# Juleszwanen/oscar_mpc_planner_mr_modification

Hardware: AMD Instinct MI355X
Metric: SQP solves/s (N=20, 8 obs, 8 guesses) at 1/2/4/8 MI355X; max |x−x_ref| (higher is better)
Workload: dtype f64

## Files before the change

__graft_entry__.py:

```python
import os
import sys

ROOT = os.path.dirname(os.path.abspath(__file__))
if ROOT not in sys.path:
    sys.path.insert(0, ROOT)


def build() -> None:
    from oscar_mpc_planner_mr_modification_amd import _build

    _build.build_lib()
    for cfg in ("C2", "C5", "C3", "JS"):
        _build.build_cpp(cfg)
    from oscar_mpc_planner_mr_modification_amd.layouts import tmpc_layout
    _build.build_instance(tmpc_layout(N=25, max_obstacles=3, name="G25"), os.path.join(_build.BUILD, "G25"))
    _build.build_stage_probe()
    _build.build_mirror_probe()
    _build.build_fac_rows_probe()
    for name in _build.FAC_AB:
        _build.build_fac_ab(name)
    _build.build_tail_ab("tail_off")
    sys.path.insert(0, os.path.join(ROOT, "oracle"))
    import oracle_py

    oracle_py.build()
    import oscar_mpc_planner_mr_modification_amd
    from oscar_mpc_planner_mr_modification_amd import native


def smoke() -> None:
    import numpy as np
    import torch

    sys.path.insert(0, os.path.join(ROOT, "oracle"))
    import oracle_py
    from oscar_mpc_planner_mr_modification_amd import native
    from oscar_mpc_planner_mr_modification_amd.layouts import config_layout
    from oscar_mpc_planner_mr_modification_amd.synthetic import make_batch

    assert torch.cuda.is_available(), "smoke() needs an MI355X"
    dev = torch.device("cuda:0")
    lay = config_layout("C2")
    b = make_batch(lay, 2, 8, seed=20251212)
    pr = native.problem_from_layout(lay)
    t = lambda a: torch.from_numpy(np.ascontiguousarray(a)).to(dev)
    out = native.solve_batch_device(pr, t(b.params), t(b.warm), t(b.xinit))
    torch.cuda.synchronize()
    ref = oracle_py.Oracle(lay).solve_batch(b.params, b.warm, b.xinit)
    exit_gpu = out["exit"].cpu().numpy()
    assert np.array_equal(exit_gpu, ref["status"]), (exit_gpu, ref["status"])
    ok = exit_gpu == 1
    assert ok.any()
    dx = np.abs(out["xtraj"].cpu().numpy()[ok] - ref["xtraj"][ok]).max()
    assert dx <= 1e-4, dx
    print(f"smoke ok: {len(exit_gpu)} solves, {int(ok.sum())} successful, max|x-x_ref| = {dx:.2e}")


if __name__ == "__main__":
    build()
    if len(sys.argv) > 1 and sys.argv[1] == "smoke":
        smoke()
```

oscar_mpc_planner_mr_modification_amd/_build.py:

```python
from __future__ import annotations

import os
import subprocess

PKG = os.path.dirname(os.path.abspath(__file__))
ROOT = os.path.dirname(PKG)
CSRC = os.path.join(PKG, "csrc")
INCLUDE = os.path.join(ROOT, "include")
LIB = os.path.join(PKG, "libmpcg.so")
ARCH = os.environ.get("MPCG_OFFLOAD_ARCH", "gfx950")

SOURCES = {"mpcg_kernels.hip": [], "mpcg_prepare.hip": ["-ffp-contract=off"],
           "mpcg_inst_tmpc20.hip": [], "mpcg_inst_tmpc30.hip": [], "mpcg_inst_shmpc.hip": [],
           "mpcg_inst_bicycle.hip": [], "mpcg_inst_road.hip": []}
HEADERS = ["mpcg_device.h", "mpcg_sqp.h", "mpcg_sqp_body.inc", "mpcg_prepare.h", "mpcg_braking.h", "mpcg_bicycle.h",
           "mpcg_instance.h", "mpcg_tail.h"]
LAYERS = {
    "mpcg_fleet.h": {"sources": {"mpcg_fleet.hip": ["-ffp-contract=off"]}, "headers": ["mpcg_fleet.h"]},
    "mpcg_path.h": {"sources": {"mpcg_path.hip": ["-ffp-contract=off"]}, "headers": ["mpcg_path.h"]},
    "mpcg_guidance.h": {"sources": {"mpcg_guidance.hip": ["-ffp-contract=off"]}, "headers": ["mpcg_guidance.h"]},
    "mpcg_active.h": {"sources": {"mpcg_active.hip": ["-ffp-contract=off"]}, "headers": ["mpcg_active.h"]},
    "mpcg_road.h": {"sources": {"mpcg_road.hip": ["-ffp-contract=off"]}, "headers": ["mpcg_road.h"]},
}
LAYER_SHARED_HEADERS = ["mpcg_host.h", "mpcg_spline.h"]
HOST_SOURCES = ["host/mpcg_yaml.cpp", "host/mpcg_solver.cpp"]
HOST_HEADERS = ["mpc_planner_solver/mpcg_yaml.h", "mpc_planner_solver/mpcg_config.h", "mpc_planner_solver/state.h",
                "mpc_planner_solver/mpcg_solver_interface.h", "mpc_planner_solver/solver_interface.h"]
BUILD = os.path.join(PKG, "build")


def source_hash() -> str:
    import hashlib

    h = hashlib.sha256()
    for f in sorted(list(SOURCES) + HEADERS):
        h.update(f.encode())
        with open(os.path.join(CSRC, f), "rb") as fh:
            h.update(fh.read())
    with open(os.path.join(INCLUDE, "mpcg.h"), "rb") as fh:
        h.update(fh.read())
    h.update(repr((ARCH, sorted(SOURCES.items()))).encode())
    return h.hexdigest()


def _stale(target, deps):
    if not os.path.exists(target):
        return True
    t = os.path.getmtime(target)
    return any(os.path.getmtime(d) > t for d in deps)


def lib_sources() -> dict:
    srcs = dict(SOURCES)
    for layer in LAYERS.values():
        srcs.update(layer["sources"])
    return srcs


def build_lib(force: bool = False, verbose: bool = False, extra_flags=(), out: str = LIB, sources=None) -> str:
    srcs = {k: v for k, v in lib_sources().items() if sources is None or k not in SOURCES or k in sources}
    layer_headers = LAYER_SHARED_HEADERS + [h for layer in LAYERS.values() for h in layer["headers"]]
    deps = [os.path.join(CSRC, f) for f in list(lib_sources()) + HEADERS + layer_headers] + \
        [os.path.join(INCLUDE, h) for h in ["mpcg.h"] + list(LAYERS)] + [__file__]
    if not force and not _stale(out, deps):
        return out
    objdir = os.path.join(BUILD, "obj" + ("_" + "_".join(f.strip("-").replace("=", "") for f in extra_flags)
                                          if extra_flags else ""))
    os.makedirs(objdir, exist_ok=True)
    common = ["hipcc", f"--offload-arch={ARCH}", "-O3", "-std=c++17", "-fPIC", f"-I{INCLUDE}", f"-I{CSRC}"]
    objs, procs = [], []
    for src, flags in srcs.items():
        obj = os.path.join(objdir, src.replace(".hip", ".o"))
        cmd = common + list(flags) + list(extra_flags) + ["-c", os.path.join(CSRC, src), "-o", obj]
        if verbose:
            print(" ".join(cmd))
        procs.append(subprocess.Popen(cmd))
        objs.append(obj)
    for p in procs:
        if p.wait() != 0:
            raise subprocess.CalledProcessError(p.returncode, "hipcc")
    cmd = ["hipcc", f"--offload-arch={ARCH}", "-shared", "-fPIC", "-Wl,-soname,libmpcg.so", "-o", out + ".tmp"] + objs
    if verbose:
        print(" ".join(cmd))
    subprocess.run(cmd, check=True)
    os.replace(out + ".tmp", out)
    return out


def _hipcc_obj(src, obj, extra=()):
    cmd = ["hipcc", f"--offload-arch={ARCH}", "-O3", "-std=c++17", "-fPIC", f"-I{INCLUDE}", f"-I{CSRC}",
           *extra, "-c", src, "-o", obj]
    subprocess.run(cmd, check=True)
    return obj


def build_instance(layout, out_dir: str, force: bool = False) -> str:
    from . import codegen

    lib_mpcg = build_lib()
    os.makedirs(out_dir, exist_ok=True)
    src = os.path.join(out_dir, "mpcg_instance.hip")
    text = codegen.instance_source(layout)
    if not os.path.exists(src) or open(src).read() != text:
        with open(src, "w") as fh:
            fh.write(text)
    so = os.path.join(out_dir, f"libmpcg_inst_{layout.name}.so")
    deps = [src, lib_mpcg, os.path.join(INCLUDE, "mpcg.h")] + [os.path.join(CSRC, h) for h in HEADERS]
    if force or _stale(so, deps):
        obj = _hipcc_obj(src, os.path.join(out_dir, "mpcg_instance.o"))
        subprocess.run(["hipcc", f"--offload-arch={ARCH}", "-shared", "-fPIC", "-o", so + ".tmp", obj, f"-L{PKG}",
                        "-lmpcg", f"-Wl,-rpath,{PKG}"], check=True)
        os.replace(so + ".tmp", so)
    return so


def _build_probe(name: str, headers, force: bool) -> str:
    src = os.path.join(ROOT, "tests", "cpp", name + ".hip")
    out_dir = os.path.join(BUILD, "probe")
    so = os.path.join(out_dir, f"lib{name}.so")
    deps = [src, os.path.join(INCLUDE, "mpcg.h"), __file__] + [os.path.join(CSRC, h) for h in headers]
    if force or _stale(so, deps):
        os.makedirs(out_dir, exist_ok=True)
        obj = _hipcc_obj(src, os.path.join(out_dir, name + ".o"))
        subprocess.run(["hipcc", f"--offload-arch={ARCH}", "-shared", "-fPIC", "-o", so + ".tmp", obj], check=True)
        os.replace(so + ".tmp", so)
    return so


def build_stage_probe(force: bool = False) -> str:
    return _build_probe("stage_probe", HEADERS, force)


def build_mirror_probe(force: bool = False) -> str:
    return _build_probe("mirror_probe", ["mpcg_device.h"], force)


def build_fac_rows_probe(force: bool = False) -> str:
    return _build_probe("fac_rows_probe", ["mpcg_device.h"], force)


FAC_AB = {"fac_rows0": ["-DMPCG_FAC_INVARIANT_ROWS=0"],
          "fac_off": ["-DMPCG_FAC_INVARIANT_ROWS=0", "-DMPCG_FAC_PIVOT_SELECT=0"]}


def build_fac_ab(name: str, force: bool = False) -> str:
    out = os.path.join(BUILD, "ab", name, "libmpcg.so")
    os.makedirs(os.path.dirname(out), exist_ok=True)
    return build_lib(force=force, extra_flags=FAC_AB[name], out=out,
                     sources=("mpcg_kernels.hip", "mpcg_prepare.hip", "mpcg_inst_tmpc20.hip"))


TAIL_AB = {"tail_off": ["-DMPCG_TAIL_LEVELS=0"], "tail_poison": ["-DMPCG_LEVEL_POISON"]}


def build_tail_ab(name: str = "tail_off", force: bool = False) -> str:
    out = os.path.join(BUILD, "ab", name, "libmpcg.so")
    os.makedirs(os.path.dirname(out), exist_ok=True)
    return build_lib(force=force, extra_flags=TAIL_AB[name], out=out,
                     sources=("mpcg_kernels.hip", "mpcg_prepare.hip", "mpcg_inst_tmpc20.hip"))


def build_cpp(config="C2", force: bool = False, verbose: bool = False) -> dict:
    from . import codegen
    from .layouts import config_layout

    lay = config_layout(config) if isinstance(config, str) else config
    lib_mpcg = build_lib()
    out = os.path.join(BUILD, lay.name)
    codegen.generate(lay, out)
    so = os.path.join(out, "libmpc_planner_solver.so")
    exe = os.path.join(out, "test_solver")
    srcs = [os.path.join(CSRC, s) for s in HOST_SOURCES] + [os.path.join(out, "mpc_planner_parameters.cpp")]
    inst = os.path.join(out, "mpcg_instance.hip")
    deps = srcs + [inst] + [os.path.join(INCLUDE, h) for h in HOST_HEADERS] + \
        [os.path.join(CSRC, h) for h in HEADERS] + [os.path.join(INCLUDE, "mpcg.h"), lib_mpcg, __file__]
    inc = [f"-I{os.path.join(out, 'include')}", f"-I{INCLUDE}"]
    if force or _stale(so, deps):
        objs = []
        for src in srcs:
            obj = os.path.join(out, os.path.basename(src).replace(".cpp", ".o"))
            cmd = ["g++", "-std=c++17", "-O2", "-fPIC", "-Wall", "-Wextra"] + inc + ["-c", src, "-o", obj]
            if verbose:
                print(" ".join(cmd))
            subprocess.run(cmd, check=True)
            objs.append(obj)
        objs.append(_hipcc_obj(inst, os.path.join(out, "mpcg_instance.o")))
        cmd = ["hipcc", f"--offload-arch={ARCH}", "-shared", "-fPIC"] + objs + \
              ["-o", so + ".tmp", f"-L{PKG}", "-lmpcg", f"-Wl,-rpath,{PKG}"]
        if verbose:
            print(" ".join(cmd))
        subprocess.run(cmd, check=True)
        os.replace(so + ".tmp", so)
    test_src = os.path.join(ROOT, "tests", "cpp", "test_solver.cpp")
    if os.path.exists(test_src) and (force or _stale(exe, [test_src, so])):
        cmd = ["g++", "-std=c++17", "-O2", "-Wall", "-Wextra"] + inc + [test_src, "-o", exe, f"-L{out}",
                                                                      "-lmpc_planner_solver", f"-L{PKG}", "-lmpcg",
                                                                      f"-Wl,-rpath,{out}:{PKG}"]
        if verbose:
            print(" ".join(cmd))
        subprocess.run(cmd, check=True)
    return {"dir": out, "lib": so, "test": exe}


if __name__ == "__main__":
    print(build_lib(force=True, verbose=True))
    print(build_cpp("C2", force=True, verbose=True))
```

oscar_mpc_planner_mr_modification_amd/csrc/mpcg_instance.h:

```cpp
#pragma once
#include <hip/hip_runtime.h>

#include <atomic>
#include <cstdio>

#include "mpcg.h"
#include "mpcg_sqp.h"

extern "C" {
typedef int (*mpcg_instance_launch)(const mpcg_problem* pr, int batch, const mpcg_io* io, void* stream,
                                    unsigned long long* stamps, void* workspace);
int mpcg_register_instance(int abi_version, int model, int N, int n_lin, int n_ell, int n_scen, int nx, mpcg_instance_launch fn,
                           int qp_mem_size, long long workspace_bytes_per_solve, const char* traits);
int mpcg_rejected_instances(void);
int mpcg_debug_tail_levels(void* stream);
}
#define MPCG_QUEUE_BYTES 256

namespace mpcg {

template <class C, bool FULL, int PROF, int TAILK = 0>
int queue_grid(int batch, hipStream_t stream) {
    constexpr int MAXDEV = 64;
    static std::atomic<int> resident[MAXDEV];
    int dev = 0;
    if ((stream ? hipStreamGetDevice(stream, &dev) : hipGetDevice(&dev)) != hipSuccess || dev < 0 || dev >= MAXDEV)
        return batch;
    int r = resident[dev].load(std::memory_order_relaxed);
    if (r == 0) {
        int cus = 0, per_cu = 0;
        r = -1;
        if (hipDeviceGetAttribute(&cus, hipDeviceAttributeMultiprocessorCount, dev) == hipSuccess && cus > 0) {
            int cur = 0;
            const bool sw = hipGetDevice(&cur) == hipSuccess && cur != dev && hipSetDevice(dev) == hipSuccess;
            hipError_t e;
            if constexpr (TAILK != 0)
                e = hipOccupancyMaxActiveBlocksPerMultiprocessor(&per_cu, sqp_kernel<C, FULL, PROF, TAILK>, 64, 0);
            else
                e = hipOccupancyMaxActiveBlocksPerMultiprocessor(&per_cu, sqp_kernel<C, FULL, PROF>, 64, 0);
            if (e != hipSuccess) per_cu = 0;
            if (sw) (void)hipSetDevice(cur);
            if (per_cu > 0) r = per_cu * cus;
        }
        resident[dev].store(r, std::memory_order_relaxed);
    }
    return r > 0 && r < batch ? r : batch;
}

template <class C, bool FULL, int PROF>
void launch_kernel(const mpcg_problem* pr, int batch, const mpcg_io* io, hipStream_t st, unsigned long long* stamps,
                   double* gws, unsigned* queue) {
    hipLaunchKernelGGL((sqp_kernel<C, FULL, PROF>), dim3(queue ? queue_grid<C, FULL, PROF>(batch, st) : batch),
                       dim3(64), 0, st, *pr, batch, *io, stamps, gws, queue);
}

#ifndef MPCG_TAIL_K_GRIDS
#define MPCG_TAIL_K_GRIDS 3
#endif

template <class C, int PROF>
int launch_tail(const mpcg_problem* pr, int batch, const mpcg_io* io, hipStream_t st, unsigned long long* stamps,
                double* gws, unsigned* queue) {
    const int grid = queue ? queue_grid<C, false, PROF, 1>(batch, st) : batch;
    int k = 0;
    if (queue) {
        const int forced = mpcg_debug_tail_levels((void*)st);
        k = tail::plan_k(batch, grid, pr->sqp_iters, forced >= 0 ? forced : MPCG_TAIL_K_GRIDS * grid);
#ifdef MPCG_STAMPS
        k = 0;
#endif
        if (k > 0 && hipMemsetAsync(gws + (size_t)batch * slot_doubles<C>(), 0,
                                    (size_t)k * tail::WORDS_PER_SOLVE * sizeof(unsigned), st) != hipSuccess)
            return (int)hipGetLastError();
    }
    hipLaunchKernelGGL((sqp_kernel<C, false, PROF, 1>), dim3(grid), dim3(64), 0, st, *pr, batch, *io, stamps, gws,
                       queue, k);
    return (int)hipGetLastError();
}

template <class C>
int launch_instance(const mpcg_problem* pr, int batch, const mpcg_io* io, void* stream, unsigned long long* stamps,
                    void* workspace) {
    if ((gfh_doubles<C>() > 0 || (pr->qp_itref_corr_max > 0 && itref_doubles<C>() > 0)) && !workspace)
        return (int)hipErrorInvalidValue;
    unsigned* queue = C::QUEUE && workspace ? (unsigned*)workspace : nullptr;
    double* gws = workspace ? (double*)((char*)workspace + MPCG_QUEUE_BYTES) : nullptr;
    const hipStream_t st = (hipStream_t)stream;
    if (queue && hipMemsetAsync(queue, 0, MPCG_QUEUE_BYTES, st) != hipSuccess) return (int)hipGetLastError();
    const int prof = qp_profile_kind(*pr);
    const bool full = io->stats || io->qp_in || io->qp_out || needs_full(*pr) || prof == PROF_RUNTIME;
    if (full) {
        launch_kernel<C, true, PROF_RUNTIME>(pr, batch, io, st, stamps, gws, queue);
    } else if (prof == PROF_HPIPM) {
        if constexpr (tail_levels<C>()) return launch_tail<C, PROF_HPIPM>(pr, batch, io, st, stamps, gws, queue);
        else launch_kernel<C, false, PROF_HPIPM>(pr, batch, io, st, stamps, gws, queue);
    } else {
        launch_kernel<C, false, PROF_ROBUST>(pr, batch, io, st, stamps, gws, queue);
    }
    return (int)hipGetLastError();
}

template <class C>
const char* instance_traits() {
    static char buf[192];
    using L = LdsOf<C>;
    snprintf(buf, sizeof buf,
             "parts=%d slots=%d store_it=%d lean=%d gfh=%d fconst=%d pair=%d lds=%d strides=%d,%d,%d", C::PARTS,
             C::SLOTS, (int)C::STORE_IT, (int)lds_lean<C>(), (int)lds_gfh<C>(), (int)C::FCONST, (int)C::PAIR_CHAINS,
             (int)sizeof(L), L::DGS, L::HDS, L::PS);
    return buf;
}

template <class C>
int register_instance() {
    return mpcg_register_instance(MPCG_ABI_VERSION, C::MODEL, C::N, C::NL, C::NE, C::NS, C::NX, &launch_instance<C>, C::QPM,
                                  (long long)(ws_doubles<C>() * sizeof(double)), instance_traits<C>());
}

}

#define MPCG_INST_CAT2(a, b) a##b
#define MPCG_INST_CAT(a, b) MPCG_INST_CAT2(a, b)
#define MPCG_DEFINE_INSTANCE(N_, L_, E_, S_, X_, M_)                                                  \
    static const int MPCG_INST_CAT(mpcg_instance_reg_, __COUNTER__) =                                \
        mpcg::register_instance<mpcg::Cfg<N_, L_, E_, S_, X_, M_>>();
```

oscar_mpc_planner_mr_modification_amd/csrc/mpcg_sqp.h:

```cpp
#pragma once
#include <hip/hip_runtime.h>

#include <type_traits>

#include "mpcg.h"
#include "mpcg_bicycle.h"
#include "mpcg_device.h"
#include "mpcg_tail.h"

namespace mpcg {

enum { AC_SUCCESS = 0, AC_NAN = 1, AC_MAXITER = 2, AC_MINSTEP = 3, AC_QP_FAILURE = 4 };

__host__ __device__ constexpr int imax(int a, int b) { return a > b ? a : b; }
__host__ __device__ constexpr int sym(int i, int j) { return i >= j ? i * (i + 1) / 2 + j : j * (j + 1) / 2 + i; }
__host__ __device__ constexpr int cpk(int n, int a, int c) { return c * n - c * (c - 1) / 2 + (a - c); }

__host__ __device__ constexpr int lds_b64_cycles(int s, int off, int parts) {
    int total = 0;
    for (int half = 0; half < 2; ++half) {
        int dw[64] = {};
        int n = 0;
        for (int l = 32 * half; l < 32 * half + 32; ++l) {
            const int a = 2 * (s * (l / parts) + off * (l % parts));
// ... 20 lines not shown
        if (c < bc) { bc = c; best = s; }
    }
    return best;
}

template <int N_, int NL_, int NE_, int NS_ = 0, int NX_ = 5, int MODEL_ = 0>
struct Cfg {
    static constexpr int N = N_, NL = NL_, NE = NE_, NS = NS_, MODEL = MODEL_;
    static constexpr int NU = MODEL_ == 1 ? 3 : 2;
    static constexpr int NX = NX_, NZ = NU + NX_;
    static_assert(MODEL_ == 1 ? NX == 6 : (NX == 5 || NX == 6), "unicycle (+ slack state) or bicycle");
    static constexpr int IX = NU, IY = NU + 1, IPSI = NU + 2;
    static constexpr bool HAS_SLACK = MODEL_ == 1 || NX > 5;
    static constexpr int ZSL = MODEL_ == 1 ? 2 : NU + 5;
    static constexpr int NLO = NU * (NU - 1) / 2, NLC = NU == 2 ? 4 : NLO + NU;
    __host__ __device__ static constexpr int lo_idx(int i, int j) { return i * (i - 1) / 2 + j; }
    static constexpr int NH = NL + NE + NS;
    static constexpr int NTRI = NZ * (NZ + 1) / 2;
    static constexpr int NPT = NX * (NX + 1) / 2;
    static constexpr int NPTP = (MODEL_ != 1 && (64 / (N_ + 1)) >= 3) ? NPT + (NPT & 1) : NPT;
    static constexpr int NB = (HAS_SLACK && NS > 0) ? 4 : 3;
    static constexpr int NBT = NB * (NB + 1) / 2;
    static constexpr int NDH = NZ + NBT + 1;
#ifndef MPCG_PARTS_BIKE
#define MPCG_PARTS_BIKE 2
#endif
    static constexpr int PARTS_MAX = (64 / (N + 1)) >= 3 ? 3 : 2;
    static constexpr int PARTS = MODEL_ == 1 ? (MPCG_PARTS_BIKE < PARTS_MAX ? MPCG_PARTS_BIKE : PARTS_MAX) : PARTS_MAX;
    static_assert((N + 1) * PARTS <= 64, "horizon too long for one wavefront");
    static_assert(NTRI <= 64, "stage block larger than a wavefront");
    static constexpr bool QUEUE = MODEL_ == 0 && PARTS_MAX == 3;
    static constexpr int BVS = (NZ + PARTS - 1) / PARTS;
    static constexpr int HS = (NH + PARTS - 1) / PARTS;
    static constexpr int SLOTS = 2 * BVS + HS;
#ifdef MPCG_STORE_IT_ANY
    static constexpr bool STORE_IT_ANY = true;
#else
    static constexpr bool STORE_IT_ANY = false;
#endif
    static constexpr bool STORE_IT = SLOTS <= (PARTS == 3 ? 13 : STORE_IT_ANY ? 12 : 0);
    static constexpr int NBOX = 2 * NU + 2 * NX;
    static constexpr bool LIN_PARAMS = NS > 0 || N >= 30;
    static constexpr int DGC = LIN_PARAMS ? 2 : 3;
    static constexpr int NHS = LIN_PARAMS ? (NE > 0 ? NE : 1) : NH;
    static constexpr bool RELOAD_PARAMS = NS > 0 || N >= 30;
    static constexpr int M_TOTAL = 2 * NU + (N - 1) * (NBOX + NH);
    __host__ __device__ static constexpr int blk(int v) {
        return (v >= IX && v <= IPSI) ? v - IX : ((NB == 4 && v == ZSL) ? 3 : -1);
    }
    __host__ __device__ static constexpr int bvar(int b) { return b < 3 ? IX + b : ZSL; }
    static constexpr bool COMPACT = MODEL_ == 1;
    static constexpr bool FCONST = MODEL_ == 0 && N_ >= 30;
    static constexpr int NFR = COMPACT ? 4 : (FCONST ? 2 : NX), NFC = COMPACT ? NZ - 1 : NZ;
    static constexpr int NHP = COMPACT ? (NZ - 1) * NZ / 2 + 1 : NTRI;
#ifndef MPCG_FAC_INVARIANT_ROWS
#define MPCG_FAC_INVARIANT_ROWS 1
#endif
    static constexpr bool FAC_INVARIANT_ROWS =
        MPCG_FAC_INVARIANT_ROWS > 0 && MODEL_ == 0 && !FCONST && (NX_ == 5 || MPCG_FAC_INVARIANT_ROWS >= 2);
#ifndef MPCG_FAC_PIVOT_SELECT
#define MPCG_FAC_PIVOT_SELECT 1
#endif
    static constexpr bool FAC_PIVOT_SELECT =
        MPCG_FAC_PIVOT_SELECT >= 2 || (MPCG_FAC_PIVOT_SELECT == 1 && MODEL_ == 0 && !FCONST && NX_ == 5);
    static constexpr bool CHAIN_SPLIT = !COMPACT;
    static constexpr bool PAIR_WANTED = FCONST && NE_ <= 8;
    static constexpr bool PAIR_CHAINS = PAIR_WANTED && CHAIN_SPLIT && (N_ + 1) / 2 * NX_ * NX_ <= (N_ + 1) * NDH &&
                                        (N_ + 1) / 2 * NX_ <= 128;
    static constexpr bool FAC_FLAT = !COMPACT;
    static constexpr bool REC_FLAT = CHAIN_SPLIT && PARTS == 3;
#ifndef MPCG_RES_CARRY
#define MPCG_RES_CARRY 1
#endif
    static constexpr bool RES_CARRY = MPCG_RES_CARRY > 0 && MODEL_ == 0 && PARTS == 3 && NX_ == 5;
#ifndef MPCG_MIRROR_BLOCKS
#define MPCG_MIRROR_BLOCKS 1
#endif
    static constexpr bool MIRROR_BLOCKS =
        MODEL_ == 0 && (MPCG_MIRROR_BLOCKS >= 2 || (MPCG_MIRROR_BLOCKS == 1 && PARTS == 3 && NX_ == 5));
    static constexpr int QPM_ROWS = 2 * SLOTS * 64;
    static constexpr int QPM = QPM_ROWS + (N + 1) * NZ + N * NX;
    __host__ __device__ static constexpr double slack_coef(int hh) { return (NB == 4 && hh >= NL + NE) ? -1.0 : 0.0; }
};

template <class C, bool LEAN = C::COMPACT, bool GFH = false, int PAD = 0>
struct Lds {
    static constexpr int N = C::N, NX = C::NX, NZ = C::NZ;
    static constexpr int DGS =
        PAD ? lds_stride(C::NHS * C::DGC, C::DGC, C::PARTS, C::DGC % 2 == 0 ? 2 : 1, 3) : C::NHS * C::DGC;
    static constexpr int HDS = PAD ? lds_stride(C::NHS, 1, C::PARTS, 1, 3) : C::NHS;
    static constexpr int PS = PAD == 0   ? C::NPTP
                              : PAD == 2 ? lds_stride(C::NPT + (C::NPT & 1), 0, C::PARTS, 2, 4)
                                         : lds_stride(C::NPTP, 0, C::PARTS, C::NPTP == C::NPT ? 1 : 2, 4);
    double z[N + 1][NZ];
    double H[GFH ? 1 : N + 1][C::NHP];
    double g[N + 1][NZ];
    double F[GFH ? 1 : N][C::NFR][C::NFC];
    double Fst[GFH && !C::COMPACT ? C::NFR : 1][C::NFC];
    double Hst[GFH && !C::COMPACT ? C::NHP : 1];
    double b[N][NX];
    double dH[N + 1][C::NDH];
    double q[N + 1][NZ];
    double dz[N + 1][NZ];
    double ddz[N + 1][NZ];
    double pi_nlp[N][NX];
    double piq[N][NX];
    double pin[LEAN ? 1 : N][NX];
    double rdyn[LEAN ? 1 : N][NX];
    alignas(16) double P[N + 1][PS];
    double Lc[N][C::NLC];
    double Y[N][C::NU][NX];
    double bx[N + 1][NZ];
    double Dg[N][DGS];
    double hd[N][HDS];
    double disc[C::LIN_PARAMS ? N : 1][4];
    double Msc[128];
    double xinit[NX];
    int flag;
};

constexpr size_t LDS_QUARTER = 160 * 1024 / 4;
template <class C>
__host__ __device__ constexpr bool lds_lean() {
    return C::COMPACT || (sizeof(Lds<C, false>) > LDS_QUARTER && sizeof(Lds<C, true>) <= LDS_QUARTER);
}
template <class C>
__host__ __device__ constexpr bool lds_gfh() {
    return sizeof(Lds<C, lds_lean<C>(), false>) > LDS_QUARTER && sizeof(Lds<C, lds_lean<C>(), true>) <= LDS_QUARTER;
}
template <class C>
__host__ __device__ constexpr int lds_pad() {
    constexpr bool P_ALIGN = !C::COMPACT;
    return P_ALIGN && sizeof(Lds<C, lds_lean<C>(), lds_gfh<C>(), 2>) <= LDS_QUARTER ? 2
           : sizeof(Lds<C, lds_lean<C>(), lds_gfh<C>(), 1>) <= LDS_QUARTER         ? 1
                                                                                   : 0;
}
template <class C>
using LdsOf = Lds<C, lds_lean<C>(), lds_gfh<C>(), lds_pad<C>()>;
template <class C>
__host__ __device__ constexpr size_t gfh_doubles() {
    return lds_gfh<C>() ? (size_t)C::N * C::NFR * C::NFC + (size_t)(C::N + 1) * C::NHP : 0;
}
template <class C>
__host__ __device__ constexpr size_t itref_doubles() {
    return 2 * (size_t)(C::N + 1) * C::NZ + (size_t)C::N * C::NX;
}
template <class C>
__host__ __device__ constexpr size_t slot_doubles() {
    return gfh_doubles<C>() + itref_doubles<C>();
}
#ifndef MPCG_TAIL_LEVELS
#define MPCG_TAIL_LEVELS 1
#endif
template <class C>
__host__ __device__ constexpr bool tail_levels() {
    return MPCG_TAIL_LEVELS > 0 && C::QUEUE && !C::COMPACT && 2 * C::NB <= C::NZ && C::PARTS == 3 && C::NX == 5 &&
           !lds_lean<C>() && !lds_gfh<C>();
}
template <class C>
__host__ __device__ constexpr size_t carry_doubles() {
    return tail_levels<C>() ? 8 + (size_t)(C::N + 1) * C::NZ + (size_t)C::N * C::NX + 8 + 64 * (size_t)C::HS : 0;
}
template <class C>
__host__ __device__ constexpr size_t ws_doubles() {
    return slot_doubles<C>() + (tail_levels<C>() ? tail::WORDS_PER_SOLVE / 2 + carry_doubles<C>() : 0);
}

#ifdef MPCG_STAMPS
#define MPCG_NSTAMP 24
#define STAMP_DECL unsigned long long st_acc_[MPCG_NSTAMP] = {}, st_t0_ = 0, st_l_ = 0;
#define STAMP_BEGIN() do { __syncthreads(); st_t0_ = __builtin_amdgcn_s_memtime(); st_l_ = st_t0_; } while (0)
#define STAMP_END(i) do { __syncthreads(); st_acc_[i] += __builtin_amdgcn_s_memtime() - st_t0_; } while (0)
#define STAMP_LAP(i) do { const unsigned long long t_ = __builtin_amdgcn_s_memtime(); st_acc_[i] += t_ - st_l_; st_l_ = t_; } while (0)
#define STAMP_STORE(ptr, sol) \
    do { if ((ptr) && threadIdx.x == 0) for (int i_ = 0; i_ < MPCG_NSTAMP; ++i_) (ptr)[(size_t)(sol) * MPCG_NSTAMP + i_] = st_acc_[i_]; } while (0)
#elif defined(MPCG_MARKERS)
#define STAMP_DECL
#define STAMP_BEGIN() asm volatile("; @@begin")
#define STAMP_END(i) asm volatile("; @@end " #i)
#define STAMP_LAP(i) asm volatile("; @@lap " #i)
#define STAMP_STORE(ptr, sol) do {} while (0)
#else
#define STAMP_DECL
#define STAMP_BEGIN() do {} while (0)
#define STAMP_END(i) do {} while (0)
#define STAMP_LAP(i) do {} while (0)
#define STAMP_STORE(ptr, sol) do {} while (0)
#endif

__device__ __forceinline__ void wave_sync() { __asm__ volatile("" ::: "memory"); }

typedef __attribute__((address_space(3))) double lds_double;
__device__ __forceinline__ unsigned sel_lanes(unsigned long long mask, unsigned off, unsigned on) {
    unsigned r;
    asm volatile("v_cndmask_b32_e64 %0, %1, %2, %3" : "=v"(r) : "v"(off), "v"(on), "s"(mask));
    return r;
}
__device__ __forceinline__ unsigned lds_addr(double* p) { return (unsigned)(size_t)(lds_double*)p; }
__device__ __forceinline__ void lds_store(unsigned a, double v) { *(lds_double*)(size_t)a = v; }
__device__ __forceinline__ double readlane_d(double v, int lane) {
    const int lo = __builtin_amdgcn_readlane(__double2loint(v), lane);
    const int hi = __builtin_amdgcn_readlane(__double2hiint(v), lane);
    return __hiloint2double(hi, lo);
}
template <int CTRL, int ROW_MASK = 0xF>
__device__ __forceinline__ double dpp_d(double v) {
    const int lo = __builtin_amdgcn_update_dpp(__double2loint(v), __double2loint(v), CTRL, ROW_MASK, 0xF, false);
    const int hi = __builtin_amdgcn_update_dpp(__double2hiint(v), __double2hiint(v), CTRL, ROW_MASK, 0xF, false);
    return __hiloint2double(hi, lo);
}
__device__ __forceinline__ double lane_down(double v, int p) {
    double w = dpp_d<0x130>(v);
    if (p == 2) w = dpp_d<0x130>(w);
    return w;
}
__device__ __forceinline__ double wave_max(double v) {
    v = fmax(v, dpp_d<0xB1>(v));
    v = fmax(v, dpp_d<0x4E>(v));
    v = fmax(v, dpp_d<0x141>(v));
    v = fmax(v, dpp_d<0x140>(v));
    v = fmax(v, dpp_d<0x142, 0xA>(v));
    v = fmax(v, dpp_d<0x143, 0xC>(v));
    return readlane_d(v, 63);
}
__device__ __forceinline__ double wave_sum(double v) {
    v += dpp_d<0xB1>(v);
    v += dpp_d<0x4E>(v);
    v += dpp_d<0x141>(v);
    v += dpp_d<0x140>(v);
    v += dpp_d<0x142, 0xA>(v);
    v += dpp_d<0x143, 0xC>(v);
    return readlane_d(v, 63);
}


template <int n>
__device__ __forceinline__ double chain_dot(double h, const double* G, const double* v) {
    double a = h;
#pragma unroll
    for (int j = 0; j < n; ++j) a += G[j] * v[j];
    return a;
}

template <class C>
__device__ __forceinline__ double dh_at(const double* dh, int i, int j) {
    double v = (i == j) ? dh[i] : 0.0;
    const int a = C::blk(i), c = C::blk(j);
    if (a >= 0 && c >= 0) v += dh[C::NZ + (a >= c ? cpk(C::NB, a, c) : cpk(C::NB, c, a))];
    return v;
}

template <class C>
struct Rows {
    double t[C::SLOTS], l[C::SLOTS], it_[C::STORE_IT ? C::SLOTS : 1], rin[C::SLOTS], pr[C::SLOTS];
    __device__ __forceinline__ double it(int s) const {
        if constexpr (C::STORE_IT) return it_[s];
        else return frcp(t[s]);
    }
    __device__ __forceinline__ void set_it(int s, double v) {
        if constexpr (C::STORE_IT) it_[s] = v;
    }
    double nlam[C::HS];
};

template <class C>
struct LaneBounds {
    int k, part;
    double lo[C::BVS], hi[C::BVS];
    __device__ __forceinline__ double lo_at(int j) const { return lo[j]; }
    __device__ __forceinline__ double hi_at(int j) const { return hi[j]; }
};
template <class C>
struct LaneRows : LaneBounds<C> {
    using LaneBounds<C>::k;
    using LaneBounds<C>::part;
    __device__ __forceinline__ int var(int j) const { return part + C::PARTS * j; }
    __device__ __forceinline__ int hrow(int r) const { return part + C::PARTS * r; }
    __device__ __forceinline__ bool box_on(int j) const {
        const int v = var(j);
        return v < C::NZ && (k == 0 ? v < C::NU : k < C::N);
    }
    __device__ __forceinline__ bool h_on(int r) const { return k >= 1 && k < C::N && hrow(r) < C::NH; }
};

template <class C>
__device__ __forceinline__ void h_rows(const mpcg_problem& pr, const double* __restrict__ pk, const double z[C::NZ],
                                       const LaneRows<C>& LR, const double* nlam, double hb6[6],
                                       double (*Dg)[C::DGC], double* hd, double* disc) {
    const double x = z[C::IX], y = z[C::IY], psi = z[C::IPSI];
    const double rdisc = C::NE > 0 ? pk[pr.i_disc_r] : 0.0, off = pk[pr.i_disc_off];
    double sp, cp;
    sincos(psi, &sp, &cp);
    const double dxp = -off * sp, dyp = off * cp, dxpp = -off * cp, dypp = -off * sp;
    if constexpr (C::LIN_PARAMS) {
        if (LR.part == 0) { disc[0] = off * cp; disc[1] = off * sp; disc[2] = dxp; disc[3] = dyp; }
    }
#pragma unroll
    for (int r = 0; r < C::HS; ++r) {
        if (!LR.h_on(r)) continue;
        const int hh = LR.hrow(r);
        if (hh < C::NL) {
            if constexpr (!C::LIN_PARAMS) {
                const double* c = pk + pr.i_lin0 + 3 * hh;
                hd[hh] = 0.0 - (c[0] * x + c[1] * y - c[2]);
                Dg[hh][0] = c[0];
                Dg[hh][1] = c[1];
                Dg[hh][2] = 0.0;
            }
        } else if (hh >= C::NL + C::NE) {
            const double* c = pk + pr.i_scen0 + 3 * (hh - C::NL - C::NE);
            if constexpr (!C::LIN_PARAMS) {
                const double sl = C::HAS_SLACK ? z[C::ZSL] : 0.0;
                hd[hh] = 0.0 - (c[0] * (x + off * cp) + c[1] * (y + off * sp) - (c[2] + sl));
                Dg[hh][0] = c[0];
                Dg[hh][1] = c[1];
                Dg[hh][2] = c[0] * dxp + c[1] * dyp;
            }
            const double wgt = nlam[r];
            hb6[5] += wgt * (c[0] * dxpp + c[1] * dypp);
        } else {
            const double* o = pk + pr.i_ell0 + 7 * (hh - C::NL);
            const double chi = sqrt(o[5]);
            const double ra = o[3] * chi + rdisc + o[6];
            const double rb = o[4] * chi + rdisc + o[6];
            const double D0 = frcp(ra * ra), D1 = frcp(rb * rb);
            double so, co;
            sincos(o[2], &so, &co);
            const double M00 = co * co * D0 + so * so * D1;
            const double M01 = -co * so * D0 + so * co * D1;
            const double M11 = so * so * D0 + co * co * D1;
            const double ddx = x + off * cp - o[0], ddy = y + off * sp - o[1];
            const double Mdx = M00 * ddx + M01 * ddy, Mdy = M01 * ddx + M11 * ddy;
            const int he = C::LIN_PARAMS ? hh - C::NL : hh;
            hd[he] = (ddx * Mdx + ddy * Mdy) - 1.0;
            Dg[he][0] = -2.0 * Mdx;
            Dg[he][1] = -2.0 * Mdy;
            if constexpr (!C::LIN_PARAMS) Dg[he][2] = -2.0 * (Mdx * dxp + Mdy * dyp);
            const double wgt = -nlam[r];
            if (wgt != 0.0) {
                const double hxp = 2.0 * (M00 * dxp + M01 * dyp);
                const double hyp = 2.0 * (M01 * dxp + M11 * dyp);
                const double hpp = 2.0 * (dxp * (M00 * dxp + M01 * dyp) + dyp * (M01 * dxp + M11 * dyp)) +
                                   2.0 * (Mdx * dxpp + Mdy * dypp);
                hb6[0] += wgt * 2.0 * M00; hb6[1] += wgt * 2.0 * M01; hb6[2] += wgt * hxp;
                hb6[3] += wgt * 2.0 * M11; hb6[4] += wgt * hyp; hb6[5] += wgt * hpp;
            }
        }
    }
}

__host__ __device__ inline bool needs_full(const mpcg_problem& pr) {
    return pr.nlp_solver == MPCG_NLP_SQP || (pr.qp_warm_start == 2 && pr.qp_warm_first);
}

enum { PROF_RUNTIME = 0, PROF_HPIPM = 1, PROF_ROBUST = 2 };
__host__ __device__ inline int qp_profile_kind(const mpcg_problem& pr) {
    if (pr.qp_init_move == 1 && pr.qp_cond_pred_corr == 1 && pr.qp_itref_corr_max == 2 && pr.qp_sigma_clip == 0 &&
        pr.qp_maxit_first == 1 && !(pr.qp_mu_max > 0.0) && pr.qp_pivot_zero == 1)
        return PROF_HPIPM;
    if (pr.qp_init_move == 0 && pr.qp_cond_pred_corr == 0 && pr.qp_itref_corr_max == 0 && pr.qp_sigma_clip == 1 &&
        pr.qp_maxit_first == 0 && pr.qp_mu_max > 0.0 && pr.qp_pivot_zero == 0)
        return PROF_ROBUST;
    return PROF_RUNTIME;
}

#ifdef MPCG_WAVES_PER_EU
#define MPCG_KERNEL_ATTR __launch_bounds__(MPCG_WG_LANES) __attribute__((amdgpu_waves_per_eu(MPCG_WAVES_PER_EU, MPCG_WAVES_PER_EU)))
#else
#define MPCG_KERNEL_ATTR __launch_bounds__(64, 1)
#endif
struct TailDeviceAtomic {
    __host__ __device__ static unsigned fetch_add(unsigned* p, unsigned v) {
#if defined(__HIP_DEVICE_COMPILE__)
        return __hip_atomic_fetch_add(p, v, __ATOMIC_ACQ_REL, __HIP_MEMORY_SCOPE_AGENT);
#else
        const unsigned o = *p;
        *p = o + v;
        return o;
#endif
    }
};
struct TailCtl {
    int cj = 0;
    int lvl = 0;
    bool in_place = false;
};
template <int HS>
struct TailNlam {
    double v[HS];
};
template <int HS>
__device__ __attribute__((noinline)) void tail_save(double* cy, int lane, TailNlam<HS> nl, const double* z, int nz,
                                                    const double* pi, int npi, const double* xi, int nxi, int qp_total) {
    double* o = cy + 8;
    for (int e = lane; e < nz; e += 64) o[e] = z[e];
    o += nz;
    for (int e = lane; e < npi; e += 64) o[e] = pi[e];
    o += npi;
    if (lane < nxi) o[lane] = xi[lane];
    o += 8;
#pragma unroll
    for (int r = 0; r < HS; ++r) o[r * 64 + lane] = nl.v[r];
    if (lane == 0) cy[3] = qp_total;
}
template <class C, bool FULL, int PROF, bool TAIL = false>
__device__ __forceinline__ void sqp_solve(mpcg_problem pr, int batch, mpcg_io io,
                                          unsigned long long* __restrict__ stamps, double* __restrict__ gws,
                                          const int sol, const TailCtl tc, int& tail_more) {
#include "mpcg_sqp_body.inc"
}

template <class C, bool FULL = false, int PROF = PROF_RUNTIME>
__global__ MPCG_KERNEL_ATTR void sqp_kernel(mpcg_problem pr, int batch, mpcg_io io,
                                                    unsigned long long* __restrict__ stamps,
                                                    double* __restrict__ gws, unsigned* __restrict__ queue) {
    if constexpr (!C::QUEUE) {
        (void)queue;
        const int sol = blockIdx.x;
        constexpr bool TAIL = false;
        constexpr TailCtl tc{};
        [[maybe_unused]] int tail_more = 0;
#include "mpcg_sqp_body.inc"
    } else {
        if (blockDim.x != 64) {
            if (threadIdx.x == 0)
                for (int sol = blockIdx.x; sol < batch; sol += gridDim.x) io.exit_code[sol] = -1;
            return;
        }
        const bool q = queue != nullptr;
        auto next = [&]() -> int {
            unsigned t = 0;
            if (threadIdx.x == 0) t = atomicAdd(&queue[0], 1u);
            t = __builtin_amdgcn_readfirstlane(t);
            return t < (unsigned)batch ? (int)t : batch;
        };
        for (int sol = q ? next() : (int)blockIdx.x; sol < batch; sol = q ? next() : batch) {
            int more = 0;
            sqp_solve<C, FULL, PROF>(pr, batch, io, stamps, gws, sol, TailCtl{}, more);
            wave_sync();
        }
    }
}

template <class C, bool FULL, int PROF, int TAILK>
__global__ MPCG_KERNEL_ATTR void sqp_kernel(mpcg_problem pr, int batch, mpcg_io io,
                                                    unsigned long long* __restrict__ stamps,
                                                    double* __restrict__ gws, unsigned* __restrict__ queue, int tail_k) {
    static_assert(TAILK == 1 && !FULL && tail_levels<C>(), "the lean kernels of the TAIL_LEVELS instances only");
    if (blockDim.x != 64) {
        if (threadIdx.x == 0)
            for (int sol = blockIdx.x; sol < batch; sol += gridDim.x) io.exit_code[sol] = -1;
        return;
    }
    const bool q = queue != nullptr;
    auto words = [&]() { return (unsigned*)(gws + (size_t)batch * slot_doubles<C>()); };
    int sol = (int)blockIdx.x;
    int next_lvl = 0;
    for (;;) {
        TailCtl tc;
        if (next_lvl > 0) {
            tc.lvl = next_lvl;
            tc.cj = sol - (batch - tail_k) + 1;
            tc.in_place = true;
        } else if (q) {
            unsigned t = 0;
            if (threadIdx.x == 0) t = atomicAdd(&queue[0], 1u);
            t = __builtin_amdgcn_readfirstlane(t);
            const tail::Ticket tk = tail::decode(tail::Plan{batch, tail_k, pr.sqp_iters}, t);
            if (tk.kind == tail::END) break;
            sol = tk.sol;
            if (tk.kind == tail::LEVEL) {
                const int j = tk.sol - (batch - tail_k);
                unsigned mine = 0;
                if (threadIdx.x == 0) mine = tail::claim<TailDeviceAtomic>(words(), j, tk.lvl) ? 1u : 0u;
                if (!__builtin_amdgcn_readfirstlane(mine)) continue;
                __builtin_amdgcn_fence(__ATOMIC_ACQUIRE, "agent");
                tc.lvl = tk.lvl;
                tc.cj = j + 1;
            }
        }
        int more = 0;
        sqp_solve<C, FULL, PROF, true>(pr, batch, io, stamps, gws, sol, tc, more);
        wave_sync();
        if (!q) break;
        next_lvl = 0;
        if (more > 0) {
            __builtin_amdgcn_fence(__ATOMIC_RELEASE, "agent");
            unsigned go_on = 0;
            if (threadIdx.x == 0)
                go_on = tail::finish<TailDeviceAtomic>(words(), sol - (batch - tail_k), more - 1) ? 1u : 0u;
            if (__builtin_amdgcn_readfirstlane(go_on)) next_lvl = more;
        }
    }
}

}
```

oscar_mpc_planner_mr_modification_amd/csrc/mpcg_sqp_body.inc:

```
    constexpr int N = C::N, PARTS = C::PARTS, NX = C::NX, NZ = C::NZ, NB = C::NB, NBT = C::NBT;
    constexpr int NU = C::NU;
    constexpr int ZS = C::ZSL;
    constexpr int X0 = C::IX, X1 = C::IY, X2 = C::IPSI;
    constexpr bool LEAN = lds_lean<C>();
    constexpr bool GFH = lds_gfh<C>();
    constexpr bool RES_SPLIT = !C::COMPACT && 2 * NB <= NZ && PARTS == 3 && NX == 5 && !LEAN;
    constexpr int DRS = (NX + PARTS - 1) / PARTS;
    constexpr bool RES_CARRY = C::RES_CARRY && RES_SPLIT && !LEAN;
    constexpr bool CFLAG = !LEAN && !C::HAS_SLACK;
    __shared__ LdsOf<C> S;
    if (sol >= batch) return;
    if (blockDim.x != 64) {
        if (threadIdx.x == 0) io.exit_code[sol] = -1;
        return;
    }
#ifdef MPCG_LDS_POISON
    for (int e = threadIdx.x; e < (int)(sizeof(S) / 8); e += 64) ((double*)&S)[e] = __builtin_nan("");
    wave_sync();
#endif
    int lane_ = threadIdx.x;
    if constexpr (C::QUEUE) __asm__ volatile("" : "+v"(lane_));
    const int lane = lane_;
    const int k = lane / PARTS;
    const int part = lane - k * PARTS;
// ... 1939 lines not shown
                                if (stage_lane && k < N) {
#pragma unroll
                                    for (int i = 0; i < NX; ++i) pint[k * NX + i] = pinr[i];
                                }
                            }
                            wave_sync();
                            if (stage_lane) {
                                double zt[NZ];
#pragma unroll
                                for (int i = 0; i < NZ; ++i) zt[i] = S.dz[k][i] + S.ddz[k][i];
#pragma unroll
                                for (int i = 0; i < NZ; ++i) {
                                    double a = 0.0;
#pragma unroll
                                    for (int j = 0; j < NZ; ++j) a += Hat(k, i, j) * zt[j];
                                    double r = a + S.g[k][i] + S.bx[k][i];
                                    const int bi = C::blk(i);
                                    if (bi >= 0) r += ra[bi];
                                    if (k < N) {
#pragma unroll
                                        for (int m = 0; m < NX; ++m) r += Fat(k, m, i) * pint[k * NX + m];
                                    }
                                    if (k > 0 && i >= NU) r -= pint[(k - 1) * NX + i - NU];
                                    const bool free_var = (k == N) ? (i >= NU) : ((k == 0) ? (i < NU) : true);
                                    double q2 = r + S.q[k][i];
                                    if (bi >= 0) q2 += ca[bi];
                                    S.q[k][i] = free_var ? q2 : 0.0;
                                }
                                if constexpr (!LEAN) {
                                    if (k < N) {
#pragma unroll
                                        for (int i = 0; i < NX; ++i) {
                                            double a = S.b[k][i] - (S.dz[k + 1][NU + i] + S.ddz[k + 1][NU + i]);
#pragma unroll
                                            for (int j = 0; j < NZ; ++j) a += Fat(k, i, j) * zt[j];
                                            S.rdyn[k][i] = a;
                                        }
                                    }
                                }
                            }
                            {
                                ++nref;
                                for (int e = lane; e < (N + 1) * NZ; e += 64) g_ddz0[e] = (&S.ddz[0][0])[e];
                                if constexpr (LEAN) {
                                    if (stage_lane && k < N) {
#pragma unroll
                                        for (int i = 0; i < NX; ++i) g_pin0[k * NX + i] = pinr[i];
                                    }
                                    wave_sync();
                                    for (int e = lane; e < (N + 1) * NZ; e += 64) {
                                        const double d = (&S.dz[0][0])[e];
                                        g_dz0[e] = d;
                                        (&S.dz[0][0])[e] = d + (&S.ddz[0][0])[e];
                                    }
                                } else {
                                    for (int e = lane; e < N * NX; e += 64) g_pin0[e] = (&S.pin[0][0])[e];
                                }
                                redo = refining = true;
#ifdef MPCG_TRACE
                                if ((MPCG_TRACE < 0 || sol == MPCG_TRACE) && lane == 0) printf("[%d]  itref %d\n", sol, nref);
#endif
                            }
                            wave_sync();
                            if constexpr (LEAN) {
                                for (int e = lane; e <= N; e += 64) S.dH[e][C::NDH - 1] = 0.0;
                            }
                        }
                        STAMP_LAP(23);
                        alpha = 0.995 * amax;
                        if (alpha > 1.0) alpha = 1.0;
                        if (!redo && alpha >= 1e-12) {
#pragma unroll
                            for (int s = 0; s < C::SLOTS; ++s) {
                                if (!active(s)) continue;
                                double dt, dl;
                                row_step(s, dt, dl);
                                const double tn = R.t[s] + alpha * dt, ln = R.l[s] + alpha * dl;
                                R.t[s] = tn < tmin ? tmin : tn;
                                R.l[s] = ln < tmin ? tmin : ln;
                            }
                        }
                    }
                }
                wave_sync();
                STAMP_END(7);
                if (redo) {
                    redo = false;
                    phase = 0;
                }
            }
            if (qstat == AC_NAN) break;
            if (alpha < 1e-12) { qstat = AC_MINSTEP; ++qit; break; }
            STAMP_BEGIN();
            if (RES_SPLIT && !LEAN) {
                if (k <= N) {
#pragma unroll
                    for (int j = 0; j < BVS; ++j) {
                        const int v = LR.var(j);
                        if (v < NZ) S.dz[k][v] = stepped(S.dz[k][v], alpha, S.ddz[k][v]);
                    }
                    if (k < N) {
#pragma unroll
                        for (int jd = 0; jd < DRS; ++jd) {
                            const int i = part + PARTS * jd;
                            if (i < NX) {
                                const double p = S.piq[k][i];
                                S.piq[k][i] = stepped(p, alpha, S.pin[k][i] - p);
                            }
                        }
                    }
                }
            } else if (stage_lane) {
#pragma unroll
                for (int i = 0; i < NZ; ++i) S.dz[k][i] += alpha * S.ddz[k][i];
                if (k < N) {
#pragma unroll
                    for (int i = 0; i < NX; ++i) {
                        if constexpr (LEAN) S.piq[k][i] += alpha * (pinr[i] - S.piq[k][i]);
                        else S.piq[k][i] += alpha * (S.pin[k][i] - S.piq[k][i]);
                    }
                }
            }
            wave_sync();
            STAMP_END(8);
        }
        wave_sync();
        qp_status = qstat;
        qp_total += qit;
        ++sqp_iter;
        n_maxit += qstat == AC_MAXITER;
        if (qstat != AC_SUCCESS && qstat != AC_MAXITER) {
            acados_status = AC_QP_FAILURE;
            break;
        }
        if (stage_lane) {
#pragma unroll
            for (int i = 0; i < NZ; ++i) S.z[k][i] += S.dz[k][i];
            if (k == N) {
#pragma unroll
                for (int u = 0; u < NU; ++u) S.z[N][u] = 0.0;
            }
            if (k < N) {
#pragma unroll
                for (int i = 0; i < NX; ++i) S.pi_nlp[k][i] = S.piq[k][i];
            }
        }
#pragma unroll
        for (int r = 0; r < HS; ++r)
            if (LR.h_on(r)) R.nlam[r] = R.l[HB + r];
        wave_sync();
        acados_status = AC_SUCCESS;
        if (!sqp_mode && qstat != AC_SUCCESS) break;
        if constexpr (TAIL) {
            if (by_levels) break;
        }
    }
    if constexpr (TAIL) {
        if (by_levels && qp_status == AC_SUCCESS && sqp_iter < pr.sqp_iters) {
            TailNlam<HS> nl;
#pragma unroll
            for (int r = 0; r < HS; ++r) nl.v[r] = R.nlam[r];
            tail_save<HS>(carry_block(), lane, nl, &S.z[0][0], (N + 1) * NZ, &S.pi_nlp[0][0], N * NX, &S.xinit[0], NX,
                          qp_total);
            tail_more = sqp_iter;
            return;
        }
    }

    double Lk = 0.0;
    if (stage_lane && k < N) {
        double zz[NZ], gd[NZ], Hd[NZ][NZ];
#pragma unroll
        for (int i = 0; i < NZ; ++i) zz[i] = S.z[k][i];
        if constexpr (C::MODEL == 1) Lk = bike::stage_cost(pr, pk, k, zz, gd, Hd, false);
        else Lk = stage_cost<NX>(pr, pk, zz, gd, Hd, false);
    }
    const double pobj = wave_sum(Lk);
    double* xo = io.xtraj + (size_t)sol * (N + 1) * NX;
    for (int e = lane; e < (N + 1) * NX; e += 64) xo[e] = S.z[e / NX][NU + e % NX];
    double* uo = io.utraj + (size_t)sol * N * NU;
    for (int e = lane; e < N * NU; e += 64) uo[e] = S.z[e / NU][e % NU];
    if (io.lam_out) {
        double* lo = io.lam_out + (size_t)sol * N * LAMS;
        for (int e = lane; e < N * NX; e += 64) lo[(size_t)(e / NX) * LAMS + e % NX] = S.pi_nlp[e / NX][e % NX];
        if (k == 0) {
            for (int r = part; r < C::NH; r += PARTS) lo[NX + r] = 0.0;
        } else if (k < N) {
#pragma unroll
            for (int r = 0; r < HS; ++r)
                if (LR.h_on(r)) lo[(size_t)k * LAMS + NX + LR.hrow(r)] = R.nlam[r];
        }
    }
    if (FULL && io.qp_out) {
        double* q = io.qp_out + (size_t)sol * C::QPM;
#pragma unroll
        for (int sl = 0; sl < C::SLOTS; ++sl) {
            q[(2 * sl) * 64 + lane] = R.t[sl];
            q[(2 * sl + 1) * 64 + lane] = R.l[sl];
        }
        for (int e = lane; e < (N + 1) * NZ; e += 64) q[C::QPM_ROWS + e] = (&S.dz[0][0])[e];
        for (int e = lane; e < N * NX; e += 64) q[C::QPM_ROWS + (N + 1) * NZ + e] = (&S.piq[0][0])[e];
    }
    if (FULL && io.stats && lane == 0) {
        double* st = io.stats + (size_t)sol * MPCG_STATS_STRIDE;
        st[0] = nlp_stat;
        st[1] = res_eq;
        st[2] = nlp_ineq;
        st[3] = nlp_comp;
    }
    if (lane == 0) {
        int code = acados_status;
        if (res_eq > pr.res_eq_fail && code == AC_SUCCESS) code = AC_QP_FAILURE;
        if (code == AC_SUCCESS) code = 1;
        else if (code == 1) code = 0;
        io.exit_code[sol] = code;
        io.pobj[sol] = pobj;
        if (io.info) {
            io.info[(size_t)sol * MPCG_INFO_STRIDE + 0] = sqp_iter;
            io.info[(size_t)sol * MPCG_INFO_STRIDE + 1] = qp_total;
            io.info[(size_t)sol * MPCG_INFO_STRIDE + 2] = qp_status;
            io.info[(size_t)sol * MPCG_INFO_STRIDE + 3] = n_maxit;
        }
    }
    STAMP_STORE(stamps, sol);
```

oscar_mpc_planner_mr_modification_amd/csrc/mpcg_tail.h:

```cpp
#pragma once

#if defined(__HIPCC__)
#define MPCG_TAIL_HD __host__ __device__
#else
#define MPCG_TAIL_HD
#endif

namespace mpcg {
namespace tail {

constexpr int MAX_LEVELS = 16;
constexpr int WORDS_PER_SOLVE = 16;

struct Plan {
    int batch;
    int K;
    int L;
};

enum Kind { WHOLE = 0, LEVEL = 1, END = 2 };
struct Ticket {
    int kind;
    int sol;
    int lvl;
};

MPCG_TAIL_HD inline int plan_k(int batch, int grid, int levels, int want) {
    if (batch <= grid || levels > MAX_LEVELS || levels < 2 || want <= 0) return 0;
    return want < batch ? want : batch;
}

MPCG_TAIL_HD inline Ticket decode(const Plan& p, unsigned t) {
    const unsigned D = (unsigned)(p.batch - p.K);
    if (t < D) return Ticket{WHOLE, (int)t, 0};
    if (p.K <= 0 || (unsigned long long)t - D >= (unsigned long long)p.L * (unsigned)p.K) return Ticket{END, p.batch, 0};
    const unsigned r = t - D, l = r / (unsigned)p.K, j = r - l * (unsigned)p.K;
    return Ticket{LEVEL, (int)(D + j), (int)l};
}

MPCG_TAIL_HD inline unsigned word_index(int j, int l) { return (unsigned)j * WORDS_PER_SOLVE + (unsigned)l; }

template <class Atomic>
MPCG_TAIL_HD inline bool claim(unsigned* words, int j, int l) {
    if (l == 0) return true;
    return Atomic::fetch_add(&words[word_index(j, l - 1)], 1u) == 1u;
}

template <class Atomic>
MPCG_TAIL_HD inline bool finish(unsigned* words, int j, int l) {
    return Atomic::fetch_add(&words[word_index(j, l)], 1u) == 1u;
}

}
}
```

Before: 597,500.

## Group SQP tail-level tickets into multi-iteration chunks and relax claim atomics

```diff
diff --git a/__graft_entry__.py b/__graft_entry__.py
--- a/__graft_entry__.py
+++ b/__graft_entry__.py
@@ -20,6 +20,8 @@
     for name in _build.FAC_AB:
         _build.build_fac_ab(name)
     _build.build_tail_ab("tail_off")
+    for g in _build.TAIL_GROUPS:
+        _build.build_tail_ab(f"tail_g{g}")
     sys.path.insert(0, os.path.join(ROOT, "oracle"))
     import oracle_py
 
diff --git a/oscar_mpc_planner_mr_modification_amd/_build.py b/oscar_mpc_planner_mr_modification_amd/_build.py
--- a/oscar_mpc_planner_mr_modification_amd/_build.py
+++ b/oscar_mpc_planner_mr_modification_amd/_build.py
@@ -150,7 +150,10 @@
                      sources=("mpcg_kernels.hip", "mpcg_prepare.hip", "mpcg_inst_tmpc20.hip"))
 
 
-TAIL_AB = {"tail_off": ["-DMPCG_TAIL_LEVELS=0"], "tail_poison": ["-DMPCG_LEVEL_POISON"]}
+TAIL_GROUPS = (1, 2, 3)
+TAIL_AB = {"tail_off": ["-DMPCG_TAIL_LEVELS=0"], "tail_poison": ["-DMPCG_LEVEL_POISON"],
+           **{f"tail_g{g}": [f"-DMPCG_TAIL_GROUP={g}"] for g in TAIL_GROUPS},
+           "tail_fences0": ["-DMPCG_TAIL_FENCE_PAIR=0", "-DMPCG_TAIL_GROUP=1"]}
 
 
 def build_tail_ab(name: str = "tail_off", force: bool = False) -> str:
diff --git a/oscar_mpc_planner_mr_modification_amd/csrc/mpcg_instance.h b/oscar_mpc_planner_mr_modification_amd/csrc/mpcg_instance.h
--- a/oscar_mpc_planner_mr_modification_amd/csrc/mpcg_instance.h
+++ b/oscar_mpc_planner_mr_modification_amd/csrc/mpcg_instance.h
@@ -65,7 +65,8 @@
     int k = 0;
     if (queue) {
         const int forced = mpcg_debug_tail_levels((void*)st);
-        k = tail::plan_k(batch, grid, pr->sqp_iters, forced >= 0 ? forced : MPCG_TAIL_K_GRIDS * grid);
+        k = tail::plan_k(batch, grid, tail::groups(pr->sqp_iters, MPCG_TAIL_GROUP),
+                         forced >= 0 ? forced : MPCG_TAIL_K_GRIDS * grid);
 #ifdef MPCG_STAMPS
         k = 0;
 #endif
diff --git a/oscar_mpc_planner_mr_modification_amd/csrc/mpcg_sqp.h b/oscar_mpc_planner_mr_modification_amd/csrc/mpcg_sqp.h
--- a/oscar_mpc_planner_mr_modification_amd/csrc/mpcg_sqp.h
+++ b/oscar_mpc_planner_mr_modification_amd/csrc/mpcg_sqp.h
@@ -196,6 +196,13 @@
 #ifndef MPCG_TAIL_LEVELS
 #define MPCG_TAIL_LEVELS 1
 #endif
+#ifndef MPCG_TAIL_FENCE_PAIR
+#define MPCG_TAIL_FENCE_PAIR 1
+#endif
+#ifndef MPCG_TAIL_GROUP
+#define MPCG_TAIL_GROUP 2
+#endif
+static_assert(MPCG_TAIL_GROUP >= 1, "MPCG_TAIL_GROUP: SQP-RTI iterations per ticket");
 template <class C>
 __host__ __device__ constexpr bool tail_levels() {
     return MPCG_TAIL_LEVELS > 0 && C::QUEUE && !C::COMPACT && 2 * C::NB <= C::NZ && C::PARTS == 3 && C::NX == 5 &&
@@ -416,7 +423,8 @@
 struct TailDeviceAtomic {
     __host__ __device__ static unsigned fetch_add(unsigned* p, unsigned v) {
 #if defined(__HIP_DEVICE_COMPILE__)
-        return __hip_atomic_fetch_add(p, v, __ATOMIC_ACQ_REL, __HIP_MEMORY_SCOPE_AGENT);
+        return __hip_atomic_fetch_add(p, v, MPCG_TAIL_FENCE_PAIR ? __ATOMIC_RELAXED : __ATOMIC_ACQ_REL,
+                                      __HIP_MEMORY_SCOPE_AGENT);
 #else
         const unsigned o = *p;
         *p = o + v;
@@ -497,6 +505,7 @@
         return;
     }
     const bool q = queue != nullptr;
+    constexpr int G = MPCG_TAIL_GROUP;
     auto words = [&]() { return (unsigned*)(gws + (size_t)batch * slot_doubles<C>()); };
     int sol = (int)blockIdx.x;
     int next_lvl = 0;
@@ -510,7 +519,7 @@
             unsigned t = 0;
             if (threadIdx.x == 0) t = atomicAdd(&queue[0], 1u);
             t = __builtin_amdgcn_readfirstlane(t);
-            const tail::Ticket tk = tail::decode(tail::Plan{batch, tail_k, pr.sqp_iters}, t);
+            const tail::Ticket tk = tail::decode(tail::Plan{batch, tail_k, tail::groups(pr.sqp_iters, G)}, t);
             if (tk.kind == tail::END) break;
             sol = tk.sol;
             if (tk.kind == tail::LEVEL) {
@@ -519,7 +528,7 @@
                 if (threadIdx.x == 0) mine = tail::claim<TailDeviceAtomic>(words(), j, tk.lvl) ? 1u : 0u;
                 if (!__builtin_amdgcn_readfirstlane(mine)) continue;
                 __builtin_amdgcn_fence(__ATOMIC_ACQUIRE, "agent");
-                tc.lvl = tk.lvl;
+                tc.lvl = tail::group_first(tk.lvl, G);
                 tc.cj = j + 1;
             }
         }
@@ -530,9 +539,12 @@
         next_lvl = 0;
         if (more > 0) {
             __builtin_amdgcn_fence(__ATOMIC_RELEASE, "agent");
+#if MPCG_TAIL_FENCE_PAIR
+            asm volatile("s_waitcnt vmcnt(0)" ::: "memory");
+#endif
             unsigned go_on = 0;
             if (threadIdx.x == 0)
-                go_on = tail::finish<TailDeviceAtomic>(words(), sol - (batch - tail_k), more - 1) ? 1u : 0u;
+                go_on = tail::finish<TailDeviceAtomic>(words(), sol - (batch - tail_k), tail::group_of(more - 1, G)) ? 1u : 0u;
             if (__builtin_amdgcn_readfirstlane(go_on)) next_lvl = more;
         }
     }
diff --git a/oscar_mpc_planner_mr_modification_amd/csrc/mpcg_sqp_body.inc b/oscar_mpc_planner_mr_modification_amd/csrc/mpcg_sqp_body.inc
--- a/oscar_mpc_planner_mr_modification_amd/csrc/mpcg_sqp_body.inc
+++ b/oscar_mpc_planner_mr_modification_amd/csrc/mpcg_sqp_body.inc
@@ -2115,7 +2115,7 @@
         acados_status = AC_SUCCESS;
         if (!sqp_mode && qstat != AC_SUCCESS) break;
         if constexpr (TAIL) {
-            if (by_levels) break;
+            if (by_levels && tail::group_ends(it, MPCG_TAIL_GROUP)) break;
         }
     }
     if constexpr (TAIL) {
diff --git a/oscar_mpc_planner_mr_modification_amd/csrc/mpcg_tail.h b/oscar_mpc_planner_mr_modification_amd/csrc/mpcg_tail.h
--- a/oscar_mpc_planner_mr_modification_amd/csrc/mpcg_tail.h
+++ b/oscar_mpc_planner_mr_modification_amd/csrc/mpcg_tail.h
@@ -24,6 +24,11 @@
     int sol;
     int lvl;
 };
+
+MPCG_TAIL_HD constexpr int groups(int iters, int G) { return iters <= 1 ? iters : 1 + (iters - 2 + G) / G; }
+MPCG_TAIL_HD constexpr int group_first(int g, int G) { return g <= 0 ? 0 : 1 + (g - 1) * G; }
+MPCG_TAIL_HD constexpr int group_of(int it, int G) { return it <= 0 ? 0 : 1 + (it - 1) / G; }
+MPCG_TAIL_HD constexpr bool group_ends(int it, int G) { return it % G == 0; }
 
 MPCG_TAIL_HD inline int plan_k(int batch, int grid, int levels, int want) {
     if (batch <= grid || levels > MAX_LEVELS || levels < 2 || want <= 0) return 0;
```

Result: faster. 609,700 (median of 6 runs) (+2.0%).
